# SarodYatawatta/federated-pytorch-test

Measured on NVIDIA H100. Metric: train_images_per_sec, higher is better.
Workload: dtype tf32

## Files before the change

federated_pytorch_test_b200/csrc/bindings.cpp:

```cpp
#include <ATen/cuda/CUDAContext.h>
#include <c10/cuda/CUDAGuard.h>
#include <torch/extension.h>

#include <cstdlib>

#include "fedb200.h"

namespace fb = fedb200;
using torch::Tensor;

static cudaStream_t cur_stream() { return at::cuda::getCurrentCUDAStream().stream(); }
static const float* fptr(const Tensor& t) { return t.data_ptr<float>(); }
static float* fptr_mut(Tensor& t) { return t.data_ptr<float>(); }
static const float* opt_ptr(const c10::optional<Tensor>& t) { return (t.has_value() && t->defined()) ? t->data_ptr<float>() : nullptr; }

#define CHECK_F32_CUDA(x) TORCH_CHECK((x).is_cuda() && (x).scalar_type() == torch::kFloat32, #x " must be a CUDA float32 tensor")
#define CHECK_CONTIG(x) TORCH_CHECK((x).is_contiguous(), #x " must be contiguous")

void adam_prox(Tensor x, Tensor g, Tensor m, Tensor v, Tensor step, double lr, double b1, double b2, double eps,
               c10::optional<Tensor> z, c10::optional<Tensor> y, double rho, double l1, double l2,
               c10::optional<Tensor> rho_dev) {
  CHECK_F32_CUDA(x); CHECK_CONTIG(x); CHECK_CONTIG(g); CHECK_CONTIG(m); CHECK_CONTIG(v);
  c10::cuda::CUDAGuard guard(x.device());
  fb::adam_prox(fptr_mut(x), fptr(g), fptr_mut(m), fptr_mut(v), step.data_ptr<int>(), (int)x.numel(), (float)lr, (float)b1,
// ... 191 lines not shown
  CHECK_F32_CUDA(w); CHECK_CONTIG(w);
  c10::cuda::CUDAGuard guard(w.device());
  auto out = torch::empty({w.size(3), w.size(1), w.size(2), w.size(0)}, w.options());
  fb::weight_krsc_flip(fptr(w), fptr_mut(out), (int)w.size(0), (int)w.size(3), (int)w.size(1), (int)w.size(2), cur_stream());
  return out;
}

Tensor convT_pack(Tensor w) {
  CHECK_F32_CUDA(w);
  TORCH_CHECK(w.dim() == 4 && w.size(2) == 4 && w.size(3) == 4, "convT_pack: ConvTranspose2d(k=4) weight expected");
  c10::cuda::CUDAGuard guard(w.device());
  auto out = torch::empty({4 * w.size(1), 3, 3, w.size(0)}, w.options().memory_format(c10::MemoryFormat::Contiguous));
  fb::convT_pack(fptr(w), fptr_mut(out), (int)w.size(0), (int)w.size(1), w.stride(0), w.stride(1), w.stride(2), w.stride(3), cur_stream());
  return out;
}

Tensor linear_tf32(Tensor x, Tensor w, c10::optional<Tensor> bias, bool act) {
  CHECK_F32_CUDA(x); CHECK_F32_CUDA(w); CHECK_CONTIG(x); CHECK_CONTIG(w);
  TORCH_CHECK(x.dim() == 2 && w.dim() == 2 && x.size(1) == w.size(1), "linear_tf32: x [M,K], w [N,K]");
  c10::cuda::CUDAGuard guard(x.device());
  const int M = (int)x.size(0), K = (int)x.size(1), N = (int)w.size(0);
  auto out = torch::empty({M, N}, x.options());
  fb::linear_tf32(fptr(x), fptr(w), opt_ptr(bias), fptr_mut(out), M, N, K, K, K, N, act ? 1 : 0, cur_stream());
  return out;
}
bool conv_supported(int64_t H_out, int64_t W_out, int64_t C_in, int64_t stride) {
  return fb::conv_geometry_supported((int)H_out, (int)W_out, (int)C_in, (int)stride);
}
int64_t conv_orientation(int64_t NB, int64_t H_out, int64_t W_out, int64_t C_out, int64_t stride) {
  return fb::pick_conv_orientation((int)NB, (int)H_out, (int)W_out, (int)C_out, (int)stride);
}
bool conv_window_reuse(int64_t H_out, int64_t W_out, int64_t C_in, int64_t C_out, int64_t kh, int64_t stride, int64_t dil) {
  return fb::conv_window_reuse((int)H_out, (int)W_out, (int)C_in, (int)C_out, (int)kh, (int)stride, (int)dil);
}
Tensor conv2d_nhwc(Tensor x, Tensor w, c10::optional<Tensor> stats, int64_t stride, int64_t pad, int64_t dil, int64_t orient) {
  CHECK_F32_CUDA(x); CHECK_F32_CUDA(w); CHECK_CONTIG(x); CHECK_CONTIG(w);
  TORCH_CHECK(x.dim() == 4 && w.dim() == 4 && x.size(3) == w.size(3), "conv2d_nhwc: x [N,H,W,Ci], w [Co,kh,kw,Ci]");
  c10::cuda::CUDAGuard guard(x.device());
  const int NB = (int)x.size(0), H = (int)x.size(1), W = (int)x.size(2), Ci = (int)x.size(3);
  const int Co = (int)w.size(0), kh = (int)w.size(1), kw = (int)w.size(2);
  const int Ho = (H + 2 * (int)pad - (int)dil * (kh - 1) - 1) / (int)stride + 1;
  const int Wo = (W + 2 * (int)pad - (int)dil * (kw - 1) - 1) / (int)stride + 1;
  auto y = torch::empty({NB, Ho, Wo, Co}, x.options());
  float* st = (stats.has_value() && stats->defined()) ? stats->data_ptr<float>() : nullptr;
  fb::conv2d_nhwc_tf32(fptr(x), fptr(w), fptr_mut(y), st, NB, H, W, Ci, Co, kh, kw, (int)stride, (int)pad, (int)dil, Ho, Wo, cur_stream(),
                       (int)orient);
  return y;
}

Tensor conv2d_nhwc_sized(Tensor x, Tensor w, c10::optional<Tensor> stats, int64_t stride, int64_t pad, int64_t dil,
                         int64_t Ho, int64_t Wo) {
  CHECK_F32_CUDA(x); CHECK_F32_CUDA(w); CHECK_CONTIG(x); CHECK_CONTIG(w);
  TORCH_CHECK(x.dim() == 4 && w.dim() == 4 && x.size(3) == w.size(3), "conv2d_nhwc: x [N,H,W,Ci], w [Co,kh,kw,Ci]");
  TORCH_CHECK(Ho > 0 && Wo > 0, "conv2d_nhwc_sized: positive output size");
  c10::cuda::CUDAGuard guard(x.device());
  const int NB = (int)x.size(0), H = (int)x.size(1), W = (int)x.size(2), Ci = (int)x.size(3);
  const int Co = (int)w.size(0), kh = (int)w.size(1), kw = (int)w.size(2);
  auto y = torch::empty({NB, Ho, Wo, Co}, x.options());
  float* st = (stats.has_value() && stats->defined()) ? stats->data_ptr<float>() : nullptr;
  fb::conv2d_nhwc_tf32(fptr(x), fptr(w), fptr_mut(y), st, NB, H, W, Ci, Co, kh, kw, (int)stride, (int)pad, (int)dil, (int)Ho,
                       (int)Wo, cur_stream());
  return y;
}

bool conv_wgrad_supported(int64_t Cx, int64_t Co, int64_t stride, int64_t Wo, int64_t Ho) {
  return fb::conv_wgrad_supported((int)Cx, (int)Co, (int)stride, (int)Wo, (int)Ho);
// ... 522 lines not shown
int64_t launch_count() { return (int64_t)fb::launch_count(); }

PYBIND11_MODULE(TORCH_EXTENSION_NAME, m) {
  m.doc() = "federated_pytorch_test_b200: hand-written sm_90a kernels";
  m.def("launch_count", &launch_count);
  m.def("adam_prox", &adam_prox);
  m.def("bump_step", &bump_step);
  m.def("l1_l2", &l1_l2);
  m.def("make_pair", &make_pair);
  m.def("welford", &welford);
  m.def("penalty_value", &penalty_value);
  m.def("penalty_grad", &penalty_grad);
  m.def("multi_dot", &multi_dot);
  m.def("lbfgs_two_loop", &lbfgs_two_loop);
  m.def("normalize_u8", &normalize_u8);
  m.def("augment_normalize_u8", &augment_normalize_u8, py::arg("u8"), py::arg("rows"), py::arg("key"), py::arg("counter"),
        py::arg("mean"), py::arg("std"), py::arg("to_nchw"));
  m.def("col_stats", &col_stats);
  m.def("head_fwd", &head_fwd);
  m.def("head_bwd", &head_bwd);
  m.def("bn_elu_fwd", &bn_elu_fwd, py::arg("y"), py::arg("stats"), py::arg("gamma"), py::arg("beta"), py::arg("residual"),
        py::arg("running_mean"), py::arg("running_var"), py::arg("eps"), py::arg("momentum"), py::arg("act"),
        py::arg("self_clean"), py::arg("use_running") = false);
  m.def("bn_elu_bwd", &bn_elu_bwd);
  m.def("avgpool_nhwc", &avgpool_nhwc);
  m.def("avgpool_nhwc_bwd", &avgpool_nhwc_bwd);
  m.def("weight_flip", &weight_flip);
  m.def("convT_pack", &convT_pack);
  m.def("linear_tf32", &linear_tf32);
  m.def("conv_supported", &conv_supported);
  m.def("conv_orientation", &conv_orientation);
  m.def("conv_window_reuse", &conv_window_reuse, py::arg("H_out"), py::arg("W_out"), py::arg("C_in"), py::arg("C_out"), py::arg("kh"),
        py::arg("stride") = 1, py::arg("dil") = 1);
  m.def("conv2d_nhwc", &conv2d_nhwc, py::arg("x"), py::arg("w"), py::arg("stats"), py::arg("stride"), py::arg("pad"), py::arg("dil"),
        py::arg("orient") = -1);
  m.def("conv2d_nhwc_sized", &conv2d_nhwc_sized);
  m.def("conv2d_nhwc_bias_act", &conv2d_nhwc_bias_act);
  m.def("conv2d_nhwc_bn_eval", &conv2d_nhwc_bn_eval);
  m.def("conv2d_nhwc_accumulate", &conv2d_nhwc_accumulate, py::arg("x"), py::arg("w"), py::arg("y"), py::arg("stride"), py::arg("pad"),
        py::arg("dil"), py::arg("orient") = -1);
  m.def("conv2d_nhwc_shuffle", &conv2d_nhwc_shuffle);
  m.def("conv_shuffle_supported", &conv_shuffle_supported);
  m.def("conv2d_nhwc_multidil", &conv2d_nhwc_multidil);
  m.def("conv_multidil_supported", &conv_multidil_supported);
  m.def("conv_wgrad", &conv_wgrad);
  m.def("conv_wgrad_supported", &conv_wgrad_supported);
  m.def("cross_entropy_fwd", &cross_entropy_fwd);
  m.def("cross_entropy_bwd", &cross_entropy_bwd);
  m.def("vae_loss_fwd", &vae_loss_fwd);
  m.def("vae_loss_bwd", &vae_loss_bwd);
  m.def("linear_f32", &linear_f32);
  m.def("linear_f32_dgrad", &linear_f32_dgrad);
  m.def("linear_f32_wgrad", &linear_f32_wgrad);
  m.def("act_bwd_bias", &act_bwd_bias);
  m.def("maxpool2x2_fwd", &maxpool2x2_fwd);
  m.def("maxpool2x2_bwd", &maxpool2x2_bwd);
  m.def("argmax_count", &argmax_count);
  m.def("info_nce_max_p", &info_nce_max_p);
  m.def("info_nce_scratch_floats", &info_nce_scratch_floats);
  m.def("info_nce_fwd", &info_nce_fwd);
  m.def("info_nce_bwd", &info_nce_bwd);
  m.def("gauss_nll_rows_fwd", &gauss_nll_rows_fwd);
  m.def("gauss_nll_rows_bwd", &gauss_nll_rows_bwd);
  m.def("smallconv_supported", &smallconv_supported);
  m.def("smallconv_fwd", &smallconv_fwd);
  m.def("smallconv_unpool_actbwd", &smallconv_unpool_actbwd);
// ... 11 lines not shown
```

federated_pytorch_test_b200/csrc/fedb200.h:

```cpp
#pragma once
#include <cuda_runtime.h>
#include <stdint.h>

namespace fedb200 {

void count_launch(int n = 1);
long long launch_count();

bool pdl_enabled();
#ifdef __CUDACC__
__device__ __forceinline__ void pdl_wait() { asm volatile("griddepcontrol.wait;" ::: "memory"); }
__device__ __forceinline__ void pdl_launch_dependents() { asm volatile("griddepcontrol.launch_dependents;" ::: "memory"); }
__device__ __forceinline__ void pdl_prologue() {
  pdl_launch_dependents();
  pdl_wait();
}
template <typename... KArgs, typename... Args>
inline cudaError_t launch_pdl(void (*kernel)(KArgs...), dim3 grid, dim3 block, size_t smem, cudaStream_t stream,
                              Args&&... args) {
  cudaLaunchConfig_t cfg{};
  cfg.gridDim = grid;
  cfg.blockDim = block;
  cfg.dynamicSmemBytes = smem;
  cfg.stream = stream;
  cudaLaunchAttribute attr[1];
  attr[0].id = cudaLaunchAttributeProgrammaticStreamSerialization;
  attr[0].val.programmaticStreamSerializationAllowed = pdl_enabled() ? 1 : 0;
  cfg.attrs = attr;
  cfg.numAttrs = 1;
  return cudaLaunchKernelEx(&cfg, kernel, KArgs(args)...);
}
#endif

int pick_block_n(int M, int N);
void linear_tf32(const float* x, const float* w, const float* bias, float* out, int M, int N, int K, int ldx, int ldw,
                 int ldo, int act, cudaStream_t stream);
bool conv_geometry_supported(int H_out, int W_out, int C_in, int stride);
enum { CONV_ORIENT_AUTO = -1, CONV_ORIENT_ROW = 0, CONV_ORIENT_PIXEL = 1, CONV_ORIENT_PIXEL_PERTAP = 2 };
int pick_conv_orientation(int NB, int H_out, int W_out, int C_out, int stride);
bool conv_window_reuse(int H_out, int W_out, int C_in, int C_out, int kh, int stride, int dil);
void conv2d_nhwc_tf32(const float* x, const float* w, float* y, float* stats, int NB, int H, int W, int C_in, int C_out,
                      int kh, int kw, int stride, int pad, int dil, int H_out, int W_out, cudaStream_t stream,
                      int orient = CONV_ORIENT_AUTO);
void conv2d_nhwc_accumulate_tf32(const float* x, const float* w, float* y, int NB, int H, int W, int C_in, int C_out, int kh,
                                 int kw, int stride, int pad, int dil, int H_out, int W_out, cudaStream_t stream,
                                 int orient = CONV_ORIENT_AUTO);
void conv2d_nhwc_bias_act_tf32(const float* x, const float* w, const float* bias, int act, float* y, int NB, int H, int W,
                               int C_in, int C_out, int kh, int kw, int stride, int pad, int dil, int H_out, int W_out,
                               cudaStream_t stream);
void conv2d_nhwc_bn_eval_tf32(const float* x, const float* w, const float* gamma, const float* beta, const float* mean,
                              const float* var, float eps, const float* residual, int act, float* y, int NB, int H, int W,
                              int C_in, int C_out, int kh, int kw, int stride, int pad, int dil, int H_out, int W_out,
                              cudaStream_t stream);

bool conv_shuffle_supported(int H_out, int W_out, int C_in, int Ci_out);
void conv2d_nhwc_shuffle_tf32(const float* x, const float* w, float* out, int NB, int H, int W, int C_in, int C4, int kh, int kw,
                              int pad, int H_out, int W_out, cudaStream_t stream);
bool conv_multidil_supported(int H_out, int W_out, int C_in, int stride, int branches);
void conv2d_nhwc_multidil_tf32(const float* x, const float* w, const float* bias, int act, float* y, int NB, int H, int W, int C_in,
                               int C_out, int branches, int kh, int kw, int stride, const int* dils, const int* pads, int H_out,
                               int W_out, cudaStream_t stream);
bool conv_wgrad_supported(int C_x, int C_out, int stride, int W_out, int H_out);
void conv_wgrad_tf32(const float* x, const float* dy, float* dw, int NB, int H, int W, int C_x, int C_w, int C_out, int kh,
                     int kw, int stride, int pad, int dil, int H_out, int W_out, cudaStream_t stream);


void adam_prox(float* x, const float* g, float* m, float* v, const int* step_dev, int n, float lr, float b1, float b2,
               float eps, const float* z, const float* y, float rho, float l1, float l2, cudaStream_t s,
               const float* rho_dev = nullptr);
void bump_step(int* step_dev, cudaStream_t s);
void l1_l2(const float* g, int n, float* out2, cudaStream_t s);
void make_pair(const float* g, const float* gprev, const float* d, float t, float trust, float* y, float* sv, int n,
// ... 188 lines not shown
```

federated_pytorch_test_b200/csrc/gemm_wgmma.cu:

```cuda
#include "fedb200.h"
#include "igemm_wgmma.cuh"
#include "wgrad_wgmma.cuh"

#include <algorithm>
#include <cstdlib>
#include <mutex>
#include <stdexcept>
#include <string>

namespace fedb200 {

typedef CUresult (*EncodeTiledFn)(CUtensorMap*, CUtensorMapDataType, cuuint32_t, void*, const cuuint64_t*,
                                  const cuuint64_t*, const cuuint32_t*, const cuuint32_t*, CUtensorMapInterleave,
                                  CUtensorMapSwizzle, CUtensorMapL2promotion, CUtensorMapFloatOOBfill);

static EncodeTiledFn encode_fn() {
  static EncodeTiledFn fn = nullptr;
  static std::once_flag once;
  std::call_once(once, [] {
    void* p = nullptr;
    cudaDriverEntryPointQueryResult q;
    cudaError_t e = cudaGetDriverEntryPoint("cuTensorMapEncodeTiled", &p, cudaEnableDefault, &q);
    if (e != cudaSuccess || q != cudaDriverEntryPointSuccess || p == nullptr)
      throw std::runtime_error("fedb200: cuTensorMapEncodeTiled unavailable (no CUDA driver?)");
// ... 104 lines not shown
}
static void dispatch(int bn, const CUtensorMap& ta, const CUtensorMap& tb, const IgemmParams& p, cudaStream_t s) {
  if (p.bn_gamma != nullptr) dispatch_tile<true>(bn, ta, tb, p, s);
  else dispatch_tile<false>(bn, ta, tb, p, s);
}

constexpr int PIX_STAGES = 4;
constexpr int PIX_WIN_STAGES = 3;
constexpr int PIX_WIN_KH = 3;

template <int CO, int WIN_KH>
static void launch_pix(const CUtensorMap& ta, const CUtensorMap& tb, IgemmParams p, cudaStream_t stream) {
  constexpr bool WINDOW = WIN_KH > 0;
  static_assert(!WINDOW || CO == 64, "window reuse serves 64 output channels");
  constexpr int ST = WINDOW ? PIX_WIN_STAGES : PIX_STAGES;
  using S = PixSmem<CO, ST>;
  auto kernel = igemm_wgmma_pix_kernel<CO, ST, WIN_KH>;
  const int smem = WINDOW ? S::window_total(p.win_stage_bytes) : S::TOTAL;
  static bool configured = false;
  if (!configured) {
    cudaError_t e = cudaFuncSetAttribute(kernel, cudaFuncAttributeMaxDynamicSharedMemorySize, WINDOW ? 227 * 1024 : S::TOTAL);
    if (e != cudaSuccess) throw std::runtime_error(std::string("fedb200: cudaFuncSetAttribute(igemm_pix): ") + cudaGetErrorString(e));
    configured = true;
  }
  p.m_tiles = (p.M + PX_BLOCK_M - 1) / PX_BLOCK_M;
  p.n_tiles = 1;
  p.total_tiles = p.m_tiles;
  p.tma_store = 1;
  const CUtensorMap tc = make_tmap_out(p.out, p.M, p.N, p.ldo, 32);
  const int grid = std::min(p.total_tiles, num_sms());
  cudaError_t e = launch_pdl(kernel, dim3(grid), dim3(IG_THREADS), smem, stream, ta, tb, tc, p);
  if (e != cudaSuccess) throw std::runtime_error(std::string("fedb200: igemm_pix launch: ") + cudaGetErrorString(e));
  count_launch();
}

int pick_block_n(int M, int N) {
  (void)M;
  const int forced = env_int("FEDB200_BLOCK_N", 0);
  if (forced == 32 || forced == 64 || forced == 128) return forced;
  if (N <= 32) return 32;
  if (N <= 64) return 64;
  return 128;
}

static int pick_k_splits(int M, int N, int bn, int num_k_blocks) {
  const int ctas = ((M + IG_BLOCK_M - 1) / IG_BLOCK_M) * ((N + bn - 1) / bn);
  int splits = env_int("FEDB200_SPLITK", 0);
  if (splits <= 0) {
    const int wave = num_sms() + num_sms() / 8;
    splits = 1;
    while (splits < 8 && ctas * splits * 2 <= wave && num_k_blocks / (splits * 2) >= 6) splits *= 2;
  }
  return splits;
}

void linear_tf32(const float* x, const float* w, const float* bias, float* out, int M, int N, int K, int ldx, int ldw,
                 int ldo, int act, cudaStream_t stream) {
  if ((ldx & 3) || (ldw & 3) || (reinterpret_cast<uintptr_t>(x) & 15) || (reinterpret_cast<uintptr_t>(w) & 15))
    throw std::runtime_error("fedb200: linear_tf32 needs 16-byte aligned rows");
  const int bn = pick_block_n(M, N);
  CUtensorMap ta = make_tmap_2d(x, M, K, ldx, IG_BLOCK_M);
  CUtensorMap tb = make_tmap_2d(w, N, K, ldw, bn);
  IgemmParams p{};
  p.M = M; p.N = N;
  p.cblocks = (K + IG_BLOCK_K - 1) / IG_BLOCK_K;
  p.num_k_blocks = p.cblocks;
// ... 63 lines not shown
}

void conv2d_nhwc_bias_act_tf32(const float* x, const float* w, const float* bias, int act, float* y, int NB, int H, int W,
                               int C_in, int C_out, int kh, int kw, int stride, int pad, int dil, int H_out, int W_out,
                               cudaStream_t stream) {
  conv2d_generic(x, w, y, nullptr, bias, act, NB, H, W, C_in, C_out, kh, kw, stride, pad, dil, H_out, W_out, stream);
}

void conv2d_nhwc_accumulate_tf32(const float* x, const float* w, float* y, int NB, int H, int W, int C_in, int C_out, int kh,
                                 int kw, int stride, int pad, int dil, int H_out, int W_out, cudaStream_t stream, int orient) {
  if (orient == CONV_ORIENT_AUTO) orient = pick_conv_orientation(NB, H_out, W_out, C_out, stride);
  conv2d_generic(x, w, y, nullptr, nullptr, 0, NB, H, W, C_in, C_out, kh, kw, stride, pad, dil, H_out, W_out, stream, 1, nullptr,
                 orient);
}

void conv2d_nhwc_bn_eval_tf32(const float* x, const float* w, const float* gamma, const float* beta, const float* mean,
                              const float* var, float eps, const float* residual, int act, float* y, int NB, int H, int W,
                              int C_in, int C_out, int kh, int kw, int stride, int pad, int dil, int H_out, int W_out,
                              cudaStream_t stream) {
  const BnEvalArgs args{gamma, beta, mean, var, eps, residual};
  conv2d_generic(x, w, y, nullptr, nullptr, act, NB, H, W, C_in, C_out, kh, kw, stride, pad, dil, H_out, W_out, stream, 0, &args);
}

static int pick_tap_pack(int C_in) {
  if (env_int("FEDB200_TAP_PACK", 1) == 0 || C_in > 16 || (C_in & 3)) return IG_BLOCK_K;
  return C_in <= 8 ? 8 : 16;
}

static void conv2d_generic(const float* x, const float* w, float* y, float* stats, const float* bias, int act, int NB, int H,
                           int W, int C_in, int C_out, int kh, int kw, int stride, int pad, int dil, int H_out, int W_out,
                           cudaStream_t stream, int accumulate, const BnEvalArgs* eval_bn, int orient) {
  if (!conv_geometry_supported(H_out, W_out, C_in, stride))
    throw std::runtime_error("fedb200: conv geometry not supported by the wgmma path");
  const bool pix = orient == CONV_ORIENT_PIXEL || orient == CONV_ORIENT_PIXEL_PERTAP;
  if (pix && ((C_out != 64 && C_out != 128) || bias != nullptr || act != 0 || eval_bn != nullptr ||
              !pix_geometry_supported(H_out, W_out, stride) || (reinterpret_cast<uintptr_t>(y) & 15) != 0))
    throw std::runtime_error("fedb200: pixel-major convolution needs C_out 64 / 128, a plain, statistics or accumulate epilogue, "
                             "whole-row 256-pixel tiles and a 16-byte aligned output");
  const int win_stage = orient == CONV_ORIENT_PIXEL ? pix_window_stage_bytes(H_out, W_out, C_in, C_out, kh, stride, dil) : 0;
  const int tile_m = pix ? PX_BLOCK_M : IG_BLOCK_M;
  const int rows = tile_m / W_out;
  const int boxH = rows <= H_out ? rows : H_out;
  const int boxN = rows <= H_out ? 1 : rows / H_out;
  const int M = NB * H_out * W_out;
  const int bn = pix ? C_out : pick_block_n(M, C_out);
  const int cw = pick_tap_pack(C_in);
  CUtensorMap ta = make_tmap_nhwc(x, NB, H, W, C_in, boxN, win_stage ? boxH + kh - 1 : boxH, W_out, stride, cw);
  CUtensorMap tb = make_tmap_2d(w, C_out, uint64_t(kh) * kw * C_in, uint64_t(kh) * kw * C_in, bn, cw);
  IgemmParams p{};
  p.M = M; p.N = C_out;
  p.cblocks = (C_in + IG_BLOCK_K - 1) / IG_BLOCK_K;
  p.num_k_blocks = kh * kw * p.cblocks;
  p.taps_total = kh * kw;
  if (cw != IG_BLOCK_K) {
    p.cw = cw;
    p.num_k_blocks = (kh * kw + IG_BLOCK_K / cw - 1) / (IG_BLOCK_K / cw);
  }
  p.taps_w = kw; p.b_cols_per_tap = C_in; p.is_conv = 1;
  p.HW_out = H_out * W_out; p.W_out = W_out;
  p.stride = stride; p.pad = pad; p.dil = dil;
  p.out = y; p.ldo = C_out; p.bias = bias; p.act = act; p.stats = stats;
  p.k_splits = 1; p.kb_per_split = p.num_k_blocks;
  p.accumulate = accumulate;
  if (win_stage) {
    p.num_k_blocks = kw * p.cblocks;
    p.kb_per_split = p.num_k_blocks;
    p.win_rows = boxH + kh - 1;
    p.win_a_bytes = p.win_rows * W_out * IG_BLOCK_K * 4;
    p.win_stage_bytes = win_stage;
    launch_pix<64, PIX_WIN_KH>(ta, tb, p, stream);
    return;
  }
  if (pix) {
    if (C_out == 64) launch_pix<64, 0>(ta, tb, p, stream);
    else launch_pix<128, 0>(ta, tb, p, stream);
    return;
  }
  if (bias == nullptr && (act == 0 || eval_bn != nullptr)) {
    const int splits = pick_k_splits(M, C_out, bn, p.num_k_blocks);
    if (splits > 1) {
      p.kb_per_split = (p.num_k_blocks + splits - 1) / splits;
      p.k_splits = (p.num_k_blocks + p.kb_per_split - 1) / p.kb_per_split;
      p.stats = nullptr;
      if (!accumulate) cudaMemsetAsync(y, 0, size_t(M) * C_out * sizeof(float), stream);
    }
  }
  if (eval_bn != nullptr) {
    if ((C_out & 3) != 0) throw std::runtime_error("fedb200: eval-mode BatchNorm epilogue needs C_out % 4 == 0");
    if (p.k_splits > 1) {
      p.act = 0;
    } else {
      p.bn_gamma = eval_bn->gamma; p.bn_beta = eval_bn->beta; p.bn_mean = eval_bn->mean; p.bn_var = eval_bn->var;
      p.bn_eps = eval_bn->eps; p.residual = eval_bn->residual; p.ldr = C_out;
    }
  }
  dispatch(bn, ta, tb, p, stream);
  if (p.k_splits > 1 && stats != nullptr) col_stats(y, stats, M, C_out, stream);
  if (p.k_splits > 1 && eval_bn != nullptr)
    bn_elu_fwd(y, nullptr, eval_bn->gamma, eval_bn->beta, eval_bn->residual, y, const_cast<float*>(eval_bn->mean),
               const_cast<float*>(eval_bn->var), nullptr, nullptr, M, C_out, eval_bn->eps, 0.f, act, 0, stream, 1);
}

bool conv_shuffle_supported(int H_out, int W_out, int C_in, int Ci_out) {
  if (env_int("FEDB200_SHUFFLE_STORE", 1) == 0) return false;
  if (!conv_geometry_supported(H_out, W_out, C_in, 1)) return false;
  if (Ci_out % 32 != 0) return false;
  if (W_out > 32 || (32 % W_out) != 0) return false;
  return true;
}

// ... 145 lines not shown
```

federated_pytorch_test_b200/csrc/igemm_wgmma.cuh:

```cuda
#pragma once
#include "sm90.cuh"
#include "fedb200.h"

namespace fedb200 {

constexpr int IG_BLOCK_M = 128;
constexpr int IG_BLOCK_K = 32;
constexpr int IG_MMA_K = 8;
constexpr int IG_THREADS = 384;

struct IgemmParams {
  int M, N;
  int num_k_blocks;
  int cblocks;
  int taps_w;
  int b_cols_per_tap;
  int is_conv;
  int HW_out, W_out;
  int stride, pad, dil;
  float* out;
  int ldo;
  const float* bias;
  int act;
  float* stats;
// ... 23 lines not shown
struct IgemmSmem {
  static constexpr int A_BYTES = IG_BLOCK_M * IG_BLOCK_K * 4;
  static constexpr int B_BYTES = BLOCK_N * IG_BLOCK_K * 4;
  static constexpr int STAGE_BYTES = A_BYTES + B_BYTES;
  static constexpr int STAGING_BYTES = 2 * 64 * 32 * 4;
  static constexpr int STATS_BYTES = 2 * BLOCK_N * 4;
  static constexpr int BAR_BYTES = 2 * STAGES * 8;
  static constexpr int TOTAL = STAGES * STAGE_BYTES + STAGING_BYTES + STATS_BYTES + BAR_BYTES + 1024;
};

struct TileCoord {
  int m0, n0, kb_begin, kb_count;
};
__device__ __forceinline__ TileCoord decode_tile(const IgemmParams& p, int t, int block_m, int block_n) {
  const int n_idx = t % p.n_tiles;
  const int rest = t / p.n_tiles;
  const int m_idx = rest % p.m_tiles;
  const int z = rest / p.m_tiles;
  TileCoord c;
  c.m0 = m_idx * block_m;
  c.n0 = n_idx * block_n;
  c.kb_begin = z * p.kb_per_split;
  c.kb_count = min(p.kb_per_split, p.num_k_blocks - c.kb_begin);
  return c;
}

__device__ __forceinline__ void named_bar_sync(uint32_t id, uint32_t n) {
  asm volatile("bar.sync %0, %1;" ::"r"(id), "r"(n) : "memory");
}
__device__ __forceinline__ void named_bar_arrive(uint32_t id, uint32_t n) {
  asm volatile("bar.arrive %0, %1;" ::"r"(id), "r"(n) : "memory");
}

template <int TILE_M, int BLOCK_N, int STAGES, int A_BYTES, int STAGE_BYTES>
__device__ __forceinline__ void igemm_produce(const IgemmParams& p, uint8_t* tiles, uint64_t* full_bar, uint64_t* empty_bar,
                                              const CUtensorMap* tmap_a, const CUtensorMap* tmap_b) {
  int s = 0;
  uint32_t ph = 0;
  const int cwp = (p.cw == 8 || p.cw == 16) ? p.cw : 0;
  const int tpk = cwp ? IG_BLOCK_K / cwp : 1;
  const int img_oob = p.is_conv ? p.M / p.HW_out + 1 : 0;
  const int col_oob = p.taps_total * p.b_cols_per_tap + IG_BLOCK_K;
  auto tap_offset = [&](int rr_, int sx_, int& cw_, int& ch_) {
    cw_ = sx_ * p.dil - p.pad;
    ch_ = rr_ * p.dil;
    if (p.ms_kh > 0) {
      const int br = rr_ / p.ms_kh, rr = rr_ - br * p.ms_kh;
      const int d = int((p.ms_dil >> (8 * br)) & 0xffull), pd = int((p.ms_pad >> (8 * br)) & 0xffull);
      cw_ = sx_ * d - pd;
      ch_ = rr * d - pd;
    }
  };
  for (int t = blockIdx.x; t < p.total_tiles; t += gridDim.x) {
    const TileCoord c = decode_tile(p, t, TILE_M, BLOCK_N);
    int img = 0, h0 = 0;
    if (p.is_conv) {
      img = c.m0 / p.HW_out;
      h0 = ((c.m0 - img * p.HW_out) / p.W_out) * p.stride - p.pad;
    }
    int tap = c.kb_begin / p.cblocks;
    int cb = c.kb_begin - tap * p.cblocks;
    int r = tap / p.taps_w, sx = tap - r * p.taps_w;
    for (int kb = c.kb_begin; kb < c.kb_begin + c.kb_count; ++kb) {
      mbar_wait(&empty_bar[s], ph ^ 1);
      uint8_t* a_dst = tiles + s * STAGE_BYTES;
      uint8_t* b_dst = a_dst + A_BYTES;
      mbar_arrive_expect_tx(&full_bar[s], uint32_t(STAGE_BYTES));
      if (cwp) {
        const int sub_a = TILE_M * cwp * 4, sub_b = BLOCK_N * cwp * 4;
        for (int jt = 0; jt < tpk; ++jt) {
          const int tp = kb * tpk + jt;
          const bool real = tp < p.taps_total;
          int cw = 0, ch = 0;
          if (real) tap_offset(tp / p.taps_w, tp % p.taps_w, cw, ch);
          tma_load_4d(a_dst + jt * sub_a, tmap_a, &full_bar[s], 0, cw, h0 + ch, real ? img : img_oob);
          tma_load_2d(b_dst + jt * sub_b, tmap_b, &full_bar[s], real ? tp * p.b_cols_per_tap : col_oob, c.n0);
        }
      } else {
        int cw, ch;
        tap_offset(r, sx, cw, ch);
        if (p.is_conv)
          tma_load_4d(a_dst, tmap_a, &full_bar[s], cb * IG_BLOCK_K, cw, h0 + ch, img);
        else
          tma_load_2d(a_dst, tmap_a, &full_bar[s], kb * IG_BLOCK_K, c.m0);
        tma_load_2d(b_dst, tmap_b, &full_bar[s], (r * p.taps_w + sx) * p.b_cols_per_tap + cb * IG_BLOCK_K, c.n0);
        if (++cb == p.cblocks) {
// ... 415 lines not shown
      named_bar_sync(wg_bar, 128);
#pragma unroll
      for (int ii = 0; ii < 4; ++ii) {
        const int i = 4 * q + ii;
#pragma unroll
        for (int h = 0; h < 2; ++h) {
          const int ch = ch_lo + 8 * h;
          const int cc = ch & 31;
#pragma unroll
          for (int e = 0; e < 2; ++e) {
            const int px = 8 * ii + px_in + e;
            buf[(ch >> 5) * 1024 + px * 32 + (((uint32_t(cc) >> 2) ^ uint32_t(px & 7)) << 2) + (cc & 3)] = acc[4 * i + 2 * h + e];
          }
        }
      }
      fence_proxy_async();
      named_bar_sync(wg_bar, 128);
      if (tid == 0) {
        const int row0 = c.m0 + 32 * q;
        if (row0 < p.M) {
#pragma unroll
          for (int b = 0; b < 2; ++b) {
            if (p.accumulate) tma_reduce_add_2d(&tmap_c, buf + b * 1024, ch_wg + 32 * b, row0);
            else tma_store_2d(&tmap_c, buf + b * 1024, ch_wg + 32 * b, row0);
          }
        }
        tma_store_commit();
      }
    }
  }
  if (tid == 0) tma_store_wait_read();
}

}
```

federated_pytorch_test_b200/csrc/sm90.cuh:

```cuda
#pragma once
#include <cuda.h>
#include <cuda_runtime.h>
#include <stdint.h>

namespace fedb200 {

__device__ __forceinline__ uint32_t smem_u32(const void* p) {
  return static_cast<uint32_t>(__cvta_generic_to_shared(p));
}

__device__ __forceinline__ void mbar_init(uint64_t* bar, uint32_t count) {
  asm volatile("mbarrier.init.shared::cta.b64 [%0], %1;" ::"r"(smem_u32(bar)), "r"(count) : "memory");
}
__device__ __forceinline__ void fence_barrier_init() {
  asm volatile("fence.mbarrier_init.release.cluster;" ::: "memory");
}
__device__ __forceinline__ void fence_proxy_async() {
  asm volatile("fence.proxy.async.shared::cta;" ::: "memory");
}
__device__ __forceinline__ void mbar_arrive_expect_tx(uint64_t* bar, uint32_t bytes) {
  asm volatile("mbarrier.arrive.expect_tx.shared::cta.b64 _, [%0], %1;" ::"r"(smem_u32(bar)), "r"(bytes) : "memory");
}
__device__ __forceinline__ void mbar_arrive(uint64_t* bar) {
  asm volatile("mbarrier.arrive.shared::cta.b64 _, [%0];" ::"r"(smem_u32(bar)) : "memory");
// ... 156 lines not shown
      "}, %128, %129, p, 1, 1;\n\t}\n"
      : "+f"(d[0]), "+f"(d[1]), "+f"(d[2]), "+f"(d[3]), "+f"(d[4]), "+f"(d[5]), "+f"(d[6]), "+f"(d[7]),
        "+f"(d[8]), "+f"(d[9]), "+f"(d[10]), "+f"(d[11]), "+f"(d[12]), "+f"(d[13]), "+f"(d[14]), "+f"(d[15]),
        "+f"(d[16]), "+f"(d[17]), "+f"(d[18]), "+f"(d[19]), "+f"(d[20]), "+f"(d[21]), "+f"(d[22]), "+f"(d[23]),
        "+f"(d[24]), "+f"(d[25]), "+f"(d[26]), "+f"(d[27]), "+f"(d[28]), "+f"(d[29]), "+f"(d[30]), "+f"(d[31]),
        "+f"(d[32]), "+f"(d[33]), "+f"(d[34]), "+f"(d[35]), "+f"(d[36]), "+f"(d[37]), "+f"(d[38]), "+f"(d[39]),
        "+f"(d[40]), "+f"(d[41]), "+f"(d[42]), "+f"(d[43]), "+f"(d[44]), "+f"(d[45]), "+f"(d[46]), "+f"(d[47]),
        "+f"(d[48]), "+f"(d[49]), "+f"(d[50]), "+f"(d[51]), "+f"(d[52]), "+f"(d[53]), "+f"(d[54]), "+f"(d[55]),
        "+f"(d[56]), "+f"(d[57]), "+f"(d[58]), "+f"(d[59]), "+f"(d[60]), "+f"(d[61]), "+f"(d[62]), "+f"(d[63]),
        "+f"(d[64]), "+f"(d[65]), "+f"(d[66]), "+f"(d[67]), "+f"(d[68]), "+f"(d[69]), "+f"(d[70]), "+f"(d[71]),
        "+f"(d[72]), "+f"(d[73]), "+f"(d[74]), "+f"(d[75]), "+f"(d[76]), "+f"(d[77]), "+f"(d[78]), "+f"(d[79]),
        "+f"(d[80]), "+f"(d[81]), "+f"(d[82]), "+f"(d[83]), "+f"(d[84]), "+f"(d[85]), "+f"(d[86]), "+f"(d[87]),
        "+f"(d[88]), "+f"(d[89]), "+f"(d[90]), "+f"(d[91]), "+f"(d[92]), "+f"(d[93]), "+f"(d[94]), "+f"(d[95]),
        "+f"(d[96]), "+f"(d[97]), "+f"(d[98]), "+f"(d[99]), "+f"(d[100]), "+f"(d[101]), "+f"(d[102]), "+f"(d[103]),
        "+f"(d[104]), "+f"(d[105]), "+f"(d[106]), "+f"(d[107]), "+f"(d[108]), "+f"(d[109]), "+f"(d[110]), "+f"(d[111]),
        "+f"(d[112]), "+f"(d[113]), "+f"(d[114]), "+f"(d[115]), "+f"(d[116]), "+f"(d[117]), "+f"(d[118]), "+f"(d[119]),
        "+f"(d[120]), "+f"(d[121]), "+f"(d[122]), "+f"(d[123]), "+f"(d[124]), "+f"(d[125]), "+f"(d[126]), "+f"(d[127])
      : "l"(adesc), "l"(bdesc), "r"(accumulate));
}

template <int N>
__device__ __forceinline__ void wgmma_tf32(float (&d)[N / 2], uint64_t adesc, uint64_t bdesc, uint32_t accumulate) {
  if constexpr (N == 32) wgmma_tf32_n32(d, adesc, bdesc, accumulate);
  else if constexpr (N == 64) wgmma_tf32_n64(d, adesc, bdesc, accumulate);
  else wgmma_tf32_n128(d, adesc, bdesc, accumulate);
}


template <int N>
__device__ __forceinline__ void setmaxnreg_dec() { asm volatile("setmaxnreg.dec.sync.aligned.u32 %0;" ::"n"(N)); }
template <int N>
__device__ __forceinline__ void setmaxnreg_inc() { asm volatile("setmaxnreg.inc.sync.aligned.u32 %0;" ::"n"(N)); }

__device__ __forceinline__ float elu1(float v) { return v > 0.f ? v : (__expf(v) - 1.f); }

__device__ __forceinline__ float warp_sum(float v) {
#pragma unroll
  for (int o = 16; o > 0; o >>= 1) v += __shfl_xor_sync(0xffffffffu, v, o);
  return v;
}

}
```

Measured before the change: 35280.

## Add wide-N implicit GEMM conv kernel with cluster split-K reduction via DSMEM

Adds a new implicit-GEMM conv kernel that computes 256-wide output-channel tiles with wgmma n256, one tile per CTA. When there are too few tiles to fill the SMs, K is split across a 1/2/4-CTA thread block cluster and partial accumulators are reduced through distributed shared memory instead of global split-K. It is selected automatically for plain row-orientation convs with no bias or activation, aiming to raise SM fill and A-operand reuse for mid-sized layers. The cost is high register pressure (128 accumulators per thread), extra cluster barriers, and an occupancy heuristic that may choose the path where it does not pay off.

```diff
diff --git a/federated_pytorch_test_b200/csrc/bindings.cpp b/federated_pytorch_test_b200/csrc/bindings.cpp
--- a/federated_pytorch_test_b200/csrc/bindings.cpp
+++ b/federated_pytorch_test_b200/csrc/bindings.cpp
@@ -247,6 +247,9 @@
 }
 bool conv_window_reuse(int64_t H_out, int64_t W_out, int64_t C_in, int64_t C_out, int64_t kh, int64_t stride, int64_t dil) {
   return fb::conv_window_reuse((int)H_out, (int)W_out, (int)C_in, (int)C_out, (int)kh, (int)stride, (int)dil);
+}
+int64_t conv_wide_tile(int64_t NB, int64_t H_out, int64_t W_out, int64_t C_in, int64_t C_out, int64_t kh, int64_t stride) {
+  return fb::pick_wide_tile((int)NB, (int)H_out, (int)W_out, (int)C_in, (int)C_out, (int)kh, (int)kh, (int)stride);
 }
 Tensor conv2d_nhwc(Tensor x, Tensor w, c10::optional<Tensor> stats, int64_t stride, int64_t pad, int64_t dil, int64_t orient) {
   CHECK_F32_CUDA(x); CHECK_F32_CUDA(w); CHECK_CONTIG(x); CHECK_CONTIG(w);
@@ -835,6 +838,8 @@
   m.def("conv_orientation", &conv_orientation);
   m.def("conv_window_reuse", &conv_window_reuse, py::arg("H_out"), py::arg("W_out"), py::arg("C_in"), py::arg("C_out"), py::arg("kh"),
         py::arg("stride") = 1, py::arg("dil") = 1);
+  m.def("conv_wide_tile", &conv_wide_tile, py::arg("NB"), py::arg("H_out"), py::arg("W_out"), py::arg("C_in"), py::arg("C_out"),
+        py::arg("kh"), py::arg("stride") = 1);
   m.def("conv2d_nhwc", &conv2d_nhwc, py::arg("x"), py::arg("w"), py::arg("stats"), py::arg("stride"), py::arg("pad"), py::arg("dil"),
         py::arg("orient") = -1);
   m.def("conv2d_nhwc_sized", &conv2d_nhwc_sized);
diff --git a/federated_pytorch_test_b200/csrc/fedb200.h b/federated_pytorch_test_b200/csrc/fedb200.h
--- a/federated_pytorch_test_b200/csrc/fedb200.h
+++ b/federated_pytorch_test_b200/csrc/fedb200.h
@@ -36,8 +36,9 @@
 void linear_tf32(const float* x, const float* w, const float* bias, float* out, int M, int N, int K, int ldx, int ldw,
                  int ldo, int act, cudaStream_t stream);
 bool conv_geometry_supported(int H_out, int W_out, int C_in, int stride);
-enum { CONV_ORIENT_AUTO = -1, CONV_ORIENT_ROW = 0, CONV_ORIENT_PIXEL = 1, CONV_ORIENT_PIXEL_PERTAP = 2 };
+enum { CONV_ORIENT_AUTO = -1, CONV_ORIENT_ROW = 0, CONV_ORIENT_PIXEL = 1, CONV_ORIENT_PIXEL_PERTAP = 2, CONV_ORIENT_ROW_NARROW = 3 };
 int pick_conv_orientation(int NB, int H_out, int W_out, int C_out, int stride);
+int pick_wide_tile(int NB, int H_out, int W_out, int C_in, int C_out, int kh, int kw, int stride);
 bool conv_window_reuse(int H_out, int W_out, int C_in, int C_out, int kh, int stride, int dil);
 void conv2d_nhwc_tf32(const float* x, const float* w, float* y, float* stats, int NB, int H, int W, int C_in, int C_out,
                       int kh, int kw, int stride, int pad, int dil, int H_out, int W_out, cudaStream_t stream,
diff --git a/federated_pytorch_test_b200/csrc/gemm_wgmma.cu b/federated_pytorch_test_b200/csrc/gemm_wgmma.cu
--- a/federated_pytorch_test_b200/csrc/gemm_wgmma.cu
+++ b/federated_pytorch_test_b200/csrc/gemm_wgmma.cu
@@ -160,6 +160,90 @@
   cudaError_t e = launch_pdl(kernel, dim3(grid), dim3(IG_THREADS), smem, stream, ta, tb, tc, p);
   if (e != cudaSuccess) throw std::runtime_error(std::string("fedb200: igemm_pix launch: ") + cudaGetErrorString(e));
   count_launch();
+}
+
+template <int CL>
+static void configure_wide() {
+  static std::once_flag once;
+  std::call_once(once, [] {
+    cudaError_t e = cudaFuncSetAttribute(igemm_wgmma_wide_kernel<CL>, cudaFuncAttributeMaxDynamicSharedMemorySize, WideSmem::TOTAL);
+    if (e != cudaSuccess) throw std::runtime_error(std::string("fedb200: cudaFuncSetAttribute(igemm_wide): ") + cudaGetErrorString(e));
+  });
+}
+
+template <int CL>
+static int wide_max_clusters() {
+  static int n = -1;
+  if (n < 0) {
+    configure_wide<CL>();
+    cudaLaunchConfig_t cfg{};
+    cfg.gridDim = dim3(CL * num_sms());
+    cfg.blockDim = dim3(IG_THREADS);
+    cfg.dynamicSmemBytes = WideSmem::TOTAL;
+    cudaLaunchAttribute attr[1];
+    attr[0].id = cudaLaunchAttributeClusterDimension;
+    attr[0].val.clusterDim.x = CL;
+    attr[0].val.clusterDim.y = 1;
+    attr[0].val.clusterDim.z = 1;
+    cfg.attrs = attr;
+    cfg.numAttrs = 1;
+    int c = 0;
+    if (cudaOccupancyMaxActiveClusters(&c, igemm_wgmma_wide_kernel<CL>, &cfg) != cudaSuccess) {
+      cudaGetLastError();
+      c = 0;
+    }
+    n = c;
+  }
+  return n;
+}
+
+template <int CL>
+static void launch_wide(const CUtensorMap& ta, const CUtensorMap& tb, IgemmParams p, cudaStream_t stream) {
+  auto kernel = igemm_wgmma_wide_kernel<CL>;
+  configure_wide<CL>();
+  p.m_tiles = (p.M + IG_BLOCK_M - 1) / IG_BLOCK_M;
+  p.n_tiles = p.N / WIDE_BLOCK_N;
+  p.k_splits = CL;
+  p.kb_per_split = p.num_k_blocks / CL;
+  p.total_tiles = p.m_tiles * p.n_tiles * CL;
+  p.tma_store = 1;
+  const CUtensorMap tc = make_tmap_out(p.out, p.M, p.N, p.ldo, 32);
+  cudaLaunchConfig_t cfg{};
+  cfg.gridDim = dim3(p.total_tiles);
+  cfg.blockDim = dim3(IG_THREADS);
+  cfg.dynamicSmemBytes = WideSmem::TOTAL;
+  cfg.stream = stream;
+  cudaLaunchAttribute attr[2];
+  attr[0].id = cudaLaunchAttributeProgrammaticStreamSerialization;
+  attr[0].val.programmaticStreamSerializationAllowed = pdl_enabled() ? 1 : 0;
+  attr[1].id = cudaLaunchAttributeClusterDimension;
+  attr[1].val.clusterDim.x = CL;
+  attr[1].val.clusterDim.y = 1;
+  attr[1].val.clusterDim.z = 1;
+  cfg.attrs = attr;
+  cfg.numAttrs = CL > 1 ? 2 : 1;
+  cudaError_t e = cudaLaunchKernelEx(&cfg, kernel, ta, tb, tc, p);
+  if (e != cudaSuccess) throw std::runtime_error(std::string("fedb200: igemm_wide launch: ") + cudaGetErrorString(e));
+  count_launch();
+}
+
+constexpr int WIDE_MIN_KB = 12;
+
+int pick_wide_tile(int NB, int H_out, int W_out, int C_in, int C_out, int kh, int kw, int stride) {
+  if (env_int("FEDB200_BLOCK_N", 0) != 0 || env_int("FEDB200_SPLITK", 0) != 0) return 0;
+  if (C_out % WIDE_BLOCK_N != 0 || C_in % IG_BLOCK_K != 0 || !conv_geometry_supported(H_out, W_out, C_in, stride)) return 0;
+  const long long tiles = ((static_cast<long long>(NB) * H_out * W_out + IG_BLOCK_M - 1) / IG_BLOCK_M) * (C_out / WIDE_BLOCK_N);
+  const int kb = kh * kw * (C_in / IG_BLOCK_K);
+  const int sms = num_sms();
+  for (int s = 1; s <= 4; s *= 2) {
+    if (kb % s != 0 || kb / s < WIDE_MIN_KB) continue;
+    const long long ctas = tiles * s;
+    if (ctas > sms) break;
+    if (ctas < sms - sms / 4) continue;
+    const int resident = s == 1 ? sms : (s == 2 ? wide_max_clusters<2>() : wide_max_clusters<4>());
+    return tiles <= resident ? s : 0;
+  }
+  return 0;
 }
 
 int pick_block_n(int M, int N) {
@@ -289,6 +373,8 @@
                            cudaStream_t stream, int accumulate, const BnEvalArgs* eval_bn, int orient) {
   if (!conv_geometry_supported(H_out, W_out, C_in, stride))
     throw std::runtime_error("fedb200: conv geometry not supported by the wgmma path");
+  if (orient < CONV_ORIENT_ROW || orient > CONV_ORIENT_ROW_NARROW)
+    throw std::runtime_error("fedb200: conv orient must be -1 (auto), 0 (row), 1 (pixel), 2 (pixel, per-tap) or 3 (row, narrow)");
   const bool pix = orient == CONV_ORIENT_PIXEL || orient == CONV_ORIENT_PIXEL_PERTAP;
   if (pix && ((C_out != 64 && C_out != 128) || bias != nullptr || act != 0 || eval_bn != nullptr ||
               !pix_geometry_supported(H_out, W_out, stride) || (reinterpret_cast<uintptr_t>(y) & 15) != 0))
@@ -333,6 +419,19 @@
     else launch_pix<128, 0>(ta, tb, p, stream);
     return;
   }
+  if (orient == CONV_ORIENT_ROW && bias == nullptr && act == 0 && eval_bn == nullptr && !accumulate && cw == IG_BLOCK_K &&
+      (reinterpret_cast<uintptr_t>(y) & 15) == 0) {
+    const int cl = pick_wide_tile(NB, H_out, W_out, C_in, C_out, kh, kw, stride);
+    if (cl > 0) {
+      CUtensorMap tbw = make_tmap_2d(w, C_out, uint64_t(kh) * kw * C_in, uint64_t(kh) * kw * C_in, WIDE_BLOCK_N);
+      switch (cl) {
+        case 1: launch_wide<1>(ta, tbw, p, stream); break;
+        case 2: launch_wide<2>(ta, tbw, p, stream); break;
+        default: launch_wide<4>(ta, tbw, p, stream); break;
+      }
+      return;
+    }
+  }
   if (bias == nullptr && (act == 0 || eval_bn != nullptr)) {
     const int splits = pick_k_splits(M, C_out, bn, p.num_k_blocks);
     if (splits > 1) {
diff --git a/federated_pytorch_test_b200/csrc/igemm_wgmma.cuh b/federated_pytorch_test_b200/csrc/igemm_wgmma.cuh
--- a/federated_pytorch_test_b200/csrc/igemm_wgmma.cuh
+++ b/federated_pytorch_test_b200/csrc/igemm_wgmma.cuh
@@ -79,9 +79,9 @@
   asm volatile("bar.arrive %0, %1;" ::"r"(id), "r"(n) : "memory");
 }
 
-template <int TILE_M, int BLOCK_N, int STAGES, int A_BYTES, int STAGE_BYTES>
+template <int TILE_M, int BLOCK_N, int STAGES, int A_BYTES, int STAGE_BYTES, bool ONE_TILE = false>
 __device__ __forceinline__ void igemm_produce(const IgemmParams& p, uint8_t* tiles, uint64_t* full_bar, uint64_t* empty_bar,
-                                              const CUtensorMap* tmap_a, const CUtensorMap* tmap_b) {
+                                              const CUtensorMap* tmap_a, const CUtensorMap* tmap_b, int one_tile = 0) {
   int s = 0;
   uint32_t ph = 0;
   const int cwp = (p.cw == 8 || p.cw == 16) ? p.cw : 0;
@@ -98,7 +98,7 @@
       ch_ = rr * d - pd;
     }
   };
-  for (int t = blockIdx.x; t < p.total_tiles; t += gridDim.x) {
+  for (int t = ONE_TILE ? one_tile : int(blockIdx.x); t < p.total_tiles; t += ONE_TILE ? p.total_tiles : int(gridDim.x)) {
     const TileCoord c = decode_tile(p, t, TILE_M, BLOCK_N);
     int img = 0, h0 = 0;
     if (p.is_conv) {
@@ -580,4 +580,220 @@
   if (tid == 0) tma_store_wait_read();
 }
 
-}
+constexpr int WIDE_BLOCK_N = 256;
+template <int V>
+struct IntC {
+  static constexpr int value = V;
+};
+constexpr int WIDE_STAGES = 4;
+
+struct WideSmem {
+  static constexpr int A_BYTES = IG_BLOCK_M * IG_BLOCK_K * 4;
+  static constexpr int B_BYTES = WIDE_BLOCK_N * IG_BLOCK_K * 4;
+  static constexpr int STAGE_BYTES = A_BYTES + B_BYTES;
+  static constexpr int RING_BYTES = WIDE_STAGES * STAGE_BYTES;
+  static constexpr int STAGING_BYTES = 2 * 64 * 32 * 4;
+  static constexpr int STATS_BYTES = 8 * 2 * WIDE_BLOCK_N * 4;
+  static constexpr int BAR_BYTES = 2 * WIDE_STAGES * 8;
+  static constexpr int TOTAL = RING_BYTES + STAGING_BYTES + STATS_BYTES + BAR_BYTES + 1024;
+  static constexpr int recv_bytes(int cl) { return (cl - 1) * 256 * (WIDE_BLOCK_N / cl / 2) * 4; }
+};
+
+template <int CLUSTER>
+__global__ void __launch_bounds__(IG_THREADS, 1)
+igemm_wgmma_wide_kernel(const __grid_constant__ CUtensorMap tmap_a, const __grid_constant__ CUtensorMap tmap_b,
+                        const __grid_constant__ CUtensorMap tmap_c, const IgemmParams p) {
+  using S = WideSmem;
+  static_assert(CLUSTER == 1 || CLUSTER == 2 || CLUSTER == 4, "clusters of 1, 2 or 4 CTAs");
+  static_assert(S::TOTAL <= 227 * 1024, "shared memory budget");
+  static_assert(S::recv_bytes(CLUSTER) <= S::RING_BYTES, "the receive buffer lives in the ring");
+  static_assert(S::STAGE_BYTES % 1024 == 0, "stages must keep the 1024-byte swizzle alignment");
+  constexpr int SLICE = WIDE_BLOCK_N / CLUSTER;
+  constexpr int SLICE_ACC = SLICE / 2;
+  constexpr int QUADS = SLICE_ACC / 4;
+
+  extern __shared__ uint8_t smem_raw[];
+  uint8_t* smem = reinterpret_cast<uint8_t*>((reinterpret_cast<uintptr_t>(smem_raw) + 1023) & ~uintptr_t(1023));
+  uint8_t* tiles = smem;
+  float* staging = reinterpret_cast<float*>(smem + S::RING_BYTES);
+  float* colsum = reinterpret_cast<float*>(smem + S::RING_BYTES + S::STAGING_BYTES);
+  uint64_t* full_bar = reinterpret_cast<uint64_t*>(colsum + 8 * 2 * WIDE_BLOCK_N);
+  uint64_t* empty_bar = full_bar + WIDE_STAGES;
+
+  const int wg = threadIdx.x >> 7;
+  const int tid = threadIdx.x & 127;
+  auto my_tile = [&]() { return int(CLUSTER > 1 ? cluster_ctarank() : 0u) * (p.total_tiles / CLUSTER) + int(blockIdx.x) / CLUSTER; };
+
+  pdl_launch_dependents();
+  if (threadIdx.x == 0) {
+    tma_prefetch_desc(&tmap_a);
+    tma_prefetch_desc(&tmap_b);
+    tma_prefetch_desc(&tmap_c);
+    for (int s = 0; s < WIDE_STAGES; ++s) {
+      mbar_init(&full_bar[s], 1);
+      mbar_init(&empty_bar[s], 2);
+    }
+    fence_barrier_init();
+  }
+  __syncthreads();
+  pdl_wait();
+
+  if (wg == 0) {
+    setmaxnreg_dec<40>();
+    if (threadIdx.x == 0)
+      igemm_produce<IG_BLOCK_M, WIDE_BLOCK_N, WIDE_STAGES, S::A_BYTES, S::STAGE_BYTES, true>(p, tiles, full_bar, empty_bar,
+                                                                                             &tmap_a, &tmap_b, my_tile());
+    if constexpr (CLUSTER > 1) {
+      cluster_sync();
+      cluster_sync();
+    }
+    return;
+  }
+  setmaxnreg_inc<232>();
+
+  const int g = wg - 1;
+  const int ct = threadIdx.x - 128;
+  const int warp = tid >> 5, lane = tid & 31;
+  const uint64_t adesc0 = make_kmajor_desc(smem_u32(tiles) + uint32_t(g) * 64u * 128u, 128u);
+  const uint64_t bdesc0 = make_kmajor_desc(smem_u32(tiles) + uint32_t(S::A_BYTES), 128u);
+  float* stg = staging + g * 2048;
+  const uint32_t wg_bar = 1 + uint32_t(g);
+  const int row_in = 16 * warp + (lane >> 2);
+  const int col_in = 2 * (lane & 3);
+
+  const uint32_t rank = CLUSTER > 1 ? cluster_ctarank() : 0u;
+  const TileCoord c = decode_tile(p, my_tile(), IG_BLOCK_M, WIDE_BLOCK_N);
+  float acc[128];
+  {
+    int s = 0;
+    uint32_t ph = 0;
+    int prev = -1;
+    for (int i = 0; i < c.kb_count; ++i) {
+      mbar_wait(&full_bar[s], ph);
+      const uint64_t so = uint64_t(uint32_t(s) * uint32_t(S::STAGE_BYTES >> 4));
+      wgmma_fence();
+      wgmma_fence_acc(acc);
+#pragma unroll
+      for (int k = 0; k < IG_BLOCK_K / IG_MMA_K; ++k)
+        wgmma_tf32_n256(acc, adesc0 + so + uint32_t(2 * k), bdesc0 + so + uint32_t(2 * k), (i > 0 || k > 0) ? 1u : 0u);
+      wgmma_commit();
+      wgmma_fence_acc(acc);
+      wgmma_wait<1>();
+      if (prev >= 0 && tid == 0) mbar_arrive(&empty_bar[prev]);
+      prev = s;
+      if (++s == WIDE_STAGES) { s = 0; ph ^= 1; }
+    }
+    wgmma_wait<0>();
+    wgmma_fence_acc(acc);
+    if (prev >= 0 && tid == 0) mbar_arrive(&empty_bar[prev]);
+  }
+
+  const float4* recv = reinterpret_cast<const float4*>(tiles);
+  if constexpr (CLUSTER > 1) {
+    cluster_sync();
+#pragma unroll
+    for (int q = 0; q < CLUSTER; ++q) {
+      if (q == int(rank)) continue;
+      const int slot = int(rank) - (int(rank) > q ? 1 : 0);
+      const uint32_t dst = cluster_map_shared(smem_u32(recv + (slot * QUADS) * 256 + ct), uint32_t(q));
+#pragma unroll
+      for (int j = 0; j < QUADS; ++j) {
+        const int a = q * SLICE_ACC + 4 * j;
+        st_cluster_v4(dst + uint32_t(j) * 256u * 16u, acc[a], acc[a + 1], acc[a + 2], acc[a + 3]);
+      }
+    }
+    cluster_sync();
+  }
+
+  const int n_s = c.n0 + int(rank) * SLICE;
+  const int row_a = c.m0 + 64 * g + row_in, row_b = row_a + 8;
+  auto finish = [&](auto off) {
+    constexpr int OFF = decltype(off)::value;
+#pragma unroll
+    for (int src = 0; src < CLUSTER - 1; ++src) {
+#pragma unroll
+      for (int j = 0; j < QUADS; ++j) {
+        const float4 r = recv[(src * QUADS + j) * 256 + ct];
+        acc[OFF + 4 * j] += r.x;
+        acc[OFF + 4 * j + 1] += r.y;
+        acc[OFF + 4 * j + 2] += r.z;
+        acc[OFF + 4 * j + 3] += r.w;
+      }
+    }
+    if (row_b >= p.M) {
+      const bool ok_a = row_a < p.M;
+#pragma unroll
+      for (int i = 0; i < QUADS; ++i) {
+        if (!ok_a) { acc[OFF + 4 * i] = 0.f; acc[OFF + 4 * i + 1] = 0.f; }
+        acc[OFF + 4 * i + 2] = 0.f;
+        acc[OFF + 4 * i + 3] = 0.f;
+      }
+    }
+    if (p.stats != nullptr) {
+#pragma unroll
+      for (int i = 0; i < QUADS; ++i) {
+#pragma unroll
+        for (int e = 0; e < 2; ++e) {
+          const float va = acc[OFF + 4 * i + e], vb = acc[OFF + 4 * i + 2 + e];
+          float s1 = va + vb, s2 = fmaf(va, va, vb * vb);
+#pragma unroll
+          for (int o = 4; o < 32; o <<= 1) {
+            s1 += __shfl_xor_sync(0xffffffffu, s1, o);
+            s2 += __shfl_xor_sync(0xffffffffu, s2, o);
+          }
+          if (lane < 4) {
+            colsum[(2 * (4 * g + warp)) * SLICE + 8 * i + col_in + e] = s1;
+            colsum[(2 * (4 * g + warp) + 1) * SLICE + 8 * i + col_in + e] = s2;
+          }
+        }
+      }
+    }
+#pragma unroll
+    for (int c0 = 0; c0 < SLICE; c0 += 32) {
+      if (tid == 0) tma_store_wait_read();
+      named_bar_sync(wg_bar, 128);
+#pragma unroll
+      for (int ii = 0; ii < 4; ++ii) {
+        const int i = c0 / 8 + ii;
+        const int cc = 8 * ii + col_in;
+#pragma unroll
+        for (int h = 0; h < 2; ++h) {
+          const int r = row_in + 8 * h;
+          const int rr = r & 31;
+          float* dst = stg + (r >> 5) * 1024 + rr * 32 + (((uint32_t(cc) >> 2) ^ uint32_t(rr & 7)) << 2) + (cc & 3);
+          *reinterpret_cast<float2*>(dst) = make_float2(acc[OFF + 4 * i + 2 * h], acc[OFF + 4 * i + 2 * h + 1]);
+        }
+      }
+      fence_proxy_async();
+      named_bar_sync(wg_bar, 128);
+      if (tid == 0) {
+        for (int b = 0; b < 2; ++b) {
+          const int row0 = c.m0 + 64 * g + 32 * b;
+          if (row0 < p.M) tma_store_2d(&tmap_c, stg + b * 1024, n_s + c0, row0);
+        }
+        tma_store_commit();
+      }
+    }
+  };
+  if (rank == 0) finish(IntC<0>{});
+  if constexpr (CLUSTER >= 2) {
+    if (rank == 1) finish(IntC<SLICE_ACC>{});
+  }
+  if constexpr (CLUSTER == 4) {
+    if (rank == 2) finish(IntC<2 * SLICE_ACC>{});
+    if (rank == 3) finish(IntC<3 * SLICE_ACC>{});
+  }
+  if (p.stats != nullptr) {
+    named_bar_sync(3, 256);
+    for (int j = ct; j < 2 * SLICE; j += 256) {
+      const int k = j / SLICE, cc = j - k * SLICE;
+      float v = 0.f;
+#pragma unroll
+      for (int w = 0; w < 8; ++w) v += colsum[(2 * w + k) * SLICE + cc];
+      atomicAdd(p.stats + k * p.N + n_s + cc, v);
+    }
+  }
+  if (tid == 0) tma_store_wait_read();
+}
+
+}
diff --git a/federated_pytorch_test_b200/csrc/sm90.cuh b/federated_pytorch_test_b200/csrc/sm90.cuh
--- a/federated_pytorch_test_b200/csrc/sm90.cuh
+++ b/federated_pytorch_test_b200/csrc/sm90.cuh
@@ -212,6 +212,23 @@
 template <int N>
 __device__ __forceinline__ void setmaxnreg_inc() { asm volatile("setmaxnreg.inc.sync.aligned.u32 %0;" ::"n"(N)); }
 
+__device__ __forceinline__ uint32_t cluster_ctarank() {
+  uint32_t r;
+  asm volatile("mov.u32 %0, %%cluster_ctarank;" : "=r"(r));
+  return r;
+}
+__device__ __forceinline__ void cluster_sync() {
+  asm volatile("barrier.cluster.arrive.release;\n\tbarrier.cluster.wait.acquire;" ::: "memory");
+}
+__device__ __forceinline__ uint32_t cluster_map_shared(uint32_t smem_addr, uint32_t rank) {
+  uint32_t r;
+  asm volatile("mapa.shared::cluster.u32 %0, %1, %2;" : "=r"(r) : "r"(smem_addr), "r"(rank));
+  return r;
+}
+__device__ __forceinline__ void st_cluster_v4(uint32_t addr, float a, float b, float c, float d) {
+  asm volatile("st.shared::cluster.v4.f32 [%0], {%1, %2, %3, %4};" ::"r"(addr), "f"(a), "f"(b), "f"(c), "f"(d) : "memory");
+}
+
 __device__ __forceinline__ float elu1(float v) { return v > 0.f ? v : (__expf(v) - 1.f); }
 
 __device__ __forceinline__ float warp_sum(float v) {
```

Result: faster. 36200 (median of 6 runs) (+2.6%).
